# zamazincode/cv-diffusion-model

Measured on AMD Instinct MI355X. Metric: images/sec (whole node), 256×256 4-step LCM 'small'; PSNR vs CPU ref, higher is better.
Workload: dtype fp16; 1 GPU; variant=small, 256x256, batch=32/GPU, 4 LCM steps, fp16, 1xMI355X (BASELINE configs[1] per GPU); global_batch=32, parallelism=single GPU

## Files before the change

cv-diffusion-model_amd/_native.py:

```python
from __future__ import annotations

import ctypes as C
import os
from typing import List, Tuple

_HERE = os.path.dirname(os.path.abspath(__file__))
LIB_PATH = os.path.join(_HERE, "libllie_hip.so")

LLIE_F32, LLIE_F16, LLIE_BF16 = 0, 1, 2
LLIE_UNET, LLIE_IRB, LLIE_ATTN, LLIE_DOWN, LLIE_UP, LLIE_SE = 0, 1, 2, 3, 4, 5
ERR_ARG, ERR_SHAPE, ERR_CONFIG, ERR_KEY, ERR_NOT_LOADED, ERR_WORKSPACE, ERR_NO_DEVICE = -1, -2, -3, -4, -5, -6, -7
SAMPLER_LCM, SAMPLER_DDIM = 0, 1

EXPORTS = [
    "llie_last_error", "llie_version", "llie_create", "llie_destroy", "llie_num_params", "llie_param_info",
    "llie_load_param", "llie_params_loaded", "llie_workspace_bytes", "llie_unet_forward", "llie_module_forward",
    "llie_lcm_step", "llie_add_noise", "llie_enhance", "llie_algorithmic_bytes", "llie_flops",
    "llie_profile_begin", "llie_profile_end", "llie_enhance_workspace_bytes",
    "llie_preprocess_u8", "llie_postprocess_u8", "llie_profile_report", "llie_pw_gemm", "llie_pw_gemm_tile_rows", "llie_dwconv3x3", "llie_dwconv3x3_tiles", "llie_tune",
    "llie_grad_numel", "llie_param_grad_offset", "llie_train_workspace_bytes", "llie_unet_train_forward",
    "llie_unet_backward", "llie_module_backward", "llie_load_all", "llie_profile_dump", "llie_copy_probe", "llie_rw_probe", "llie_pw_expand", "llie_gram_stats", "llie_gram_part_floats", "llie_groupnorm_finalize", "llie_conv3x3", "llie_conv3x3_tiles", "llie_linattn", "llie_linattn_splits", "llie_se_mlp", "llie_film", "llie_refresh_params", "llie_path_bytes", "llie_time_embed", "llie_debug_irbx_stamps", "llie_debug_gemm_stamps", "llie_debug_pwx_stamps", "llie_graph_cache_entries", "llie_debug_conv_stamps", "llie_gram_finalize",
    "llie_optimizer_create", "llie_optimizer_destroy", "llie_optimizer_numel", "llie_optimizer_step",
    "llie_optimizer_step_amp",
    "llie_consistency_target", "llie_consistency_loss", "llie_ema_create", "llie_ema_update", "llie_ema_destroy",
    "llie_wgrad", "llie_wgrad_msplit", "llie_wgrad_partial_floats", "llie_dw_wgrad", "llie_dw_wgrad_strips",
    "llie_groupnorm_backward", "llie_groupnorm_backward_scratch_floats", "llie_linattn_backward", "llie_linattn_dkv_floats",
    "llie_upsample2x_backward", "llie_dilate2x", "llie_linear_dx", "llie_linear_dx_scratch_floats", "llie_linear_dw",
    "llie_final_bwd_data",
    "llie_dwconv3x3_backward", "llie_groupnorm_backward_from_slab", "llie_bias_grad", "llie_bias_grad_floats", "llie_pack_planes",
    "llie_add_into", "llie_sin_embed", "llie_pointwise_backward",
    "llie_tile_count", "llie_tile_origins", "llie_tile_gather_u8", "llie_tile_gather_f32", "llie_tile_blend_u8",
    "llie_tile_sync_step",
    "llie_aug_pair_u8", "llie_aug_synth_u8",
    "llie_image_metrics_scratch_bytes", "llie_image_metrics_f32", "llie_image_metrics_u8", "llie_comparison_grid_u8",
    "llie_upconv_fold_elems", "llie_upconv_fold_weights", "llie_conv3x3_upfold", "llie_conv3x3_upfold_tiles",
    "llie_expand_dw", "llie_expand_pool", "llie_expand_dw_project", "llie_expand_dw_project_skip", "llie_irbx_project_tiles",
    "llie_expand_stats", "llie_irbx_stats_rows",
    "llie_dwconv3x3_ex", "llie_dwconv3x3_strip_rows", "llie_last_kernel",
    "llie_init_conv", "llie_init_conv_tiles", "llie_init_conv_pack_bytes", "llie_final_conv", "llie_final_conv_pack_bytes",
    "llie_se_gate", "llie_affine_add", "llie_nchw_to_nhwc", "llie_nhwc_to_nchw", "llie_pw_gemm_dot",
    "llie_frame_shape_ok", "llie_frame_workspace_bytes", "llie_unet_forward_hw", "llie_enhance_hw",
    "llie_frame_pad", "llie_frame_load_u8", "llie_frame_store_u8",
    "llie_ssim_grad_scratch_bytes", "llie_ssim_grad_f32", "llie_x0_loss",
    "llie_train_shape_ok", "llie_unet_train_forward_hw", "llie_aug_pair_u8_hw", "llie_aug_synth_u8_hw",
    "llie_tile_gather_u8_hw", "llie_tile_gather_f32_hw", "llie_tile_blend_u8_hw", "llie_tile_sync_step_hw", "llie_frame_max_pixels",
]
K_GEMM, K_DW, K_CONV3, K_SE, K_OTHER = 1, 2, 4, 8, 16
PW_SIGMOID_BWD, PW_RELU6_BWD, PW_SILU_BWD, PW_SCALE = 0, 1, 2, 3


class GemmSeg(C.Structure):
    _fields_ = [("ptr", C.c_void_p), ("channels", C.c_int), ("scale", C.c_void_p), ("bias", C.c_void_p),
                ("affine_ld", C.c_int), ("act", C.c_int)]


class GnBackwardArgs(C.Structure):
    _fields_ = [("g", C.c_void_p), ("dz", C.c_void_p), ("x0", C.c_void_p), ("x1", C.c_void_p), ("c0", C.c_int), ("c1", C.c_int),
                ("scale", C.c_void_p), ("shift", C.c_void_p), ("act", C.c_int), ("mean", C.c_void_p), ("rstd", C.c_void_p),
                ("gamma", C.c_void_p), ("beta", C.c_void_p), ("film", C.c_void_p), ("film_stride", C.c_int64), ("dfilm", C.c_void_p),
                ("dfilm_stride", C.c_int64), ("dgamma", C.c_void_p), ("dbeta", C.c_void_p), ("add0", C.c_void_p), ("add1_0", C.c_void_p),
                ("add1_1", C.c_void_p), ("dx0", C.c_void_p), ("dx1", C.c_void_p), ("batch", C.c_int), ("pixels", C.c_int)]


class LibraryNotBuilt(RuntimeError):
    pass


class Config(C.Structure):
# ... 116 lines not shown
    L.llie_frame_workspace_bytes.restype = i64
    L.llie_unet_forward_hw.argtypes = [vp, vp, vp, vp, ci, vp, ci, ci, ci, vp, i64, vp]
    L.llie_enhance_hw.argtypes = [vp, vp, vp, vp, C.POINTER(StepCoef), ci, vp, vp, vp, ci, ci, ci, vp, i64, vp]
    L.llie_frame_pad.argtypes = [ci]
    L.llie_frame_load_u8.argtypes = [vp, ci, ci, vp, vp]
    L.llie_frame_store_u8.argtypes = [vp, ci, ci, vp, vp]
    L.llie_aug_pair_u8.argtypes = [vp, vp, ci, vp, ci, ci, ci, vp, vp, vp, vp, vp]
    L.llie_aug_synth_u8.argtypes = [vp, vp, ci, vp, ci, ci, ci, vp, vp, vp, vp, vp, vp]
    L.llie_aug_pair_u8_hw.argtypes = [vp, vp, ci, vp, ci, ci, ci, ci, vp, vp, vp, vp, vp]
    L.llie_aug_synth_u8_hw.argtypes = [vp, vp, ci, vp, ci, ci, ci, ci, vp, vp, vp, vp, vp, vp]
    L.llie_image_metrics_scratch_bytes.argtypes = [ci, ci, ci]
    L.llie_image_metrics_scratch_bytes.restype = i64
    L.llie_image_metrics_f32.argtypes = [vp, vp, ci, ci, ci, C.c_float, C.c_float, vp, vp, i64, vp]
    L.llie_image_metrics_u8.argtypes = [vp, vp, ci, ci, ci, vp, vp, i64, vp]
    L.llie_ssim_grad_scratch_bytes.argtypes = [ci, ci, ci]
    L.llie_ssim_grad_scratch_bytes.restype = i64
    L.llie_ssim_grad_f32.argtypes = [vp, vp, ci, ci, ci, C.c_float, C.c_float, vp, vp, vp, vp, i64, vp]
    L.llie_x0_loss.argtypes = [vp, vp, vp, vp, vp, ci, ci, C.c_float, C.c_float, vp, vp, ci, ci, ci, vp, i64, vp]
    L.llie_comparison_grid_u8.argtypes = [vp, vp, vp, ci, ci, ci, vp, vp]
    L.llie_pw_gemm.argtypes = [ci, C.POINTER(GemmSeg), ci, vp, vp, vp, vp, vp, ci, ci, ci, vp]
    L.llie_pw_gemm_tile_rows.argtypes = [ci]
    L.llie_pw_expand.argtypes = [ci, C.POINTER(GemmSeg), ci, vp, vp, vp, vp, ci, ci, ci, vp]
    L.llie_gram_stats.argtypes = [ci, vp, ci, vp, ci, vp, vp, ci, ci, vp, vp, vp, vp]
    L.llie_gram_part_floats.argtypes = [ci, ci]
    L.llie_gram_finalize.argtypes = [ci, vp, vp, ci, ci, vp, vp, vp, i64, C.c_float, C.c_float, ci, vp, vp, vp]
    L.llie_groupnorm_finalize.argtypes = [vp, ci, ci, vp, ci, ci, ci, ci, vp, vp, vp, i64, C.c_float, C.c_float, ci, vp, vp, vp]
    L.llie_conv3x3.argtypes = [ci, ci, vp, vp, vp, vp, vp, ci, ci, ci, ci, ci, vp]
    L.llie_conv3x3_tiles.argtypes = [ci, ci]
    L.llie_upconv_fold_elems.argtypes = [ci]
    L.llie_upconv_fold_elems.restype = i64
    L.llie_upconv_fold_weights.argtypes = [ci, vp, vp, ci, vp]
    L.llie_conv3x3_upfold.argtypes = [ci, vp, vp, vp, vp, vp, ci, ci, ci, ci, vp]
    L.llie_conv3x3_upfold_tiles.argtypes = [ci, ci]
    L.llie_linattn.argtypes = [ci, vp, vp, vp, ci, ci, ci, vp]
    L.llie_linattn_splits.argtypes = [ci]
    L.llie_se_mlp.argtypes = [ci, vp, ci, vp, vp, vp, vp, vp, vp, vp, ci, ci, ci, vp]
    L.llie_film.argtypes = [vp, vp, vp, vp, ci, ci, ci, vp]
    L.llie_gram_part_floats.restype = i64
    L.llie_dwconv3x3.argtypes = [ci, vp, vp, vp, vp, vp, vp, ci, ci, ci, ci, vp]
    L.llie_dwconv3x3_tiles.argtypes = [ci, ci]
    L.llie_dwconv3x3_ex.argtypes = [ci, vp, vp, vp, vp, vp, vp, vp, ci, ci, ci, ci, ci, vp]
    L.llie_dwconv3x3_strip_rows.argtypes = [ci, ci, ci, ci, ci]
    L.llie_init_conv_pack_bytes.argtypes = [ci, ci]
    L.llie_init_conv_pack_bytes.restype = i64
    L.llie_init_conv_tiles.argtypes = [ci, ci, ci]
    L.llie_init_conv.argtypes = [ci, vp, ci, vp, ci, vp, vp, vp, vp, ci, ci, ci, ci, ci, vp, i64, vp]
    L.llie_final_conv_pack_bytes.argtypes = [ci]
    L.llie_final_conv_pack_bytes.restype = i64
    L.llie_final_conv.argtypes = [ci, vp, vp, vp, vp, vp, vp, ci, ci, ci, ci, ci, ci, C.POINTER(StepCoef), vp, vp, vp, vp, vp, i64, vp]
    L.llie_se_gate.argtypes = [ci, vp, ci, vp, vp, vp, vp, vp, ci, ci, ci, ci, vp, vp, vp]
    L.llie_affine_add.argtypes = [ci, vp, vp, vp, vp, vp, vp, ci, ci, ci, vp]
    L.llie_nchw_to_nhwc.argtypes = [ci, vp, vp, vp, ci, ci, ci, ci, ci, vp]
    L.llie_nhwc_to_nchw.argtypes = [ci, vp, vp, ci, ci, ci, ci, ci, vp]
    L.llie_pw_gemm_dot.argtypes = [ci, C.POINTER(GemmSeg), ci, vp, vp, vp, vp, vp, ci, ci, ci, vp]
    L.llie_last_kernel.argtypes = []
    L.llie_last_kernel.restype = C.c_char_p
    L.llie_expand_dw.argtypes = [ci, vp, ci, vp, ci, vp, vp, vp, vp, vp, vp, vp, vp, ci, ci, ci, vp]
    L.llie_expand_pool.argtypes = [ci, vp, ci, vp, ci, vp, vp, vp, vp, vp, vp, vp, ci, ci, ci, vp]
    L.llie_expand_dw_project.argtypes = [ci, vp, ci, vp, vp, vp, vp, vp, vp, vp, vp, vp, vp, ci, ci, ci, vp]
    L.llie_expand_dw_project_skip.argtypes = [ci, vp, ci, vp, ci, vp, vp, vp, vp, vp, vp, vp, vp, ci, ci, vp, vp, ci, ci, ci, vp]
    L.llie_irbx_project_tiles.argtypes = [ci, ci]
    L.llie_expand_stats.argtypes = [ci, vp, ci, vp, ci, vp, vp, vp, vp, ci, ci, ci, vp]
    L.llie_irbx_stats_rows.argtypes = [ci]
    L.llie_tune.argtypes = [C.c_char_p, ci]
    L.llie_debug_irbx_stamps.argtypes = [C.POINTER(C.c_double)]
    L.llie_optimizer_create.argtypes = [C.POINTER(OptTensor), ci, C.POINTER(C.c_void_p)]
# ... 222 lines not shown
```

cv-diffusion-model_amd/csrc/engine.h:

```cpp
#pragma once
#include <hip/hip_runtime.h>

#include <algorithm>
#include <cmath>
#include <cstdarg>
#include <cstdio>
#include <cstdlib>
#include <cstring>
#include <map>
#include <tuple>
#include <string>
#include <vector>

#include "../../include/llie.h"
#include "kernels.h"

namespace llie {

void set_err(const char* fmt, ...);
inline hipStream_t hs(llie_stream stream) { return reinterpret_cast<hipStream_t>(stream); }

inline size_t elem_size(int dt) { return dt == LLIE_F32 ? 4 : 2; }
inline size_t align_up(size_t x, size_t a) { return (x + a - 1) / a * a; }

// ... 162 lines not shown
  struct GraphEntry { bool seen = false; hipGraphExec_t exec = nullptr; hipGraph_t graph = nullptr; uint64_t used = 0; };
  static constexpr size_t kMaxGraphs = 16;
  uint64_t graph_clock = 0;
  std::map<std::string, GraphEntry> graphs;
  std::map<std::tuple<int, int, int, int>, size_t> zneed;
  hipStream_t cap_stream = nullptr;
  hipStream_t side_stream = nullptr;
  hipEvent_t ev_fork = nullptr, ev_join = nullptr;
  hipStream_t branch_stream[llie::kMaxBranches] = {};
  hipEvent_t branch_join[llie::kMaxBranches] = {};
  int prof_mask = 0;
  struct ProfRec { int cls; int64_t bytes; hipEvent_t e0, e1; const char* name; char tag[56]; };
  std::vector<ProfRec> prof;
  std::vector<hipEvent_t> event_pool;
  hipEvent_t get_event() {
    if (!event_pool.empty()) { hipEvent_t e = event_pool.back(); event_pool.pop_back(); return e; }
    hipEvent_t e = nullptr;
    if (hipEventCreate(&e) != hipSuccess) return nullptr;
    return e;
  }
};

namespace llie {

struct Knobs {
  int use_irbx;
  int irbx_project;
  int gram;
  int nt_min_mb;
  int nt_mask;
  int se_mfma;
  int bwd_async;
  int upconv_fold;
  int enhance_split;
  int graph_max_steps;
  int epoch;
};
extern Knobs g_knobs;
constexpr int kGraphMaxSteps = 20;

enum IrbForm { kIrbUnfused, kIrbRecompute, kIrbProject };
struct IrbPath {
  IrbForm form;
  bool s6;
  bool fixtot;
  bool gram;
};
inline IrbPath irb_path(int dt, const IrbW& w, int c0, int H, int W, bool training) {
  IrbPath p{kIrbUnfused, !training && dt != LLIE_F32, !training && w.hid % 128 == 0, false};
  if (!p.fixtot || !g_knobs.use_irbx || w.hid != w.hid_r || w.cin != w.cin_r || !irbx_supported(dt, w.cin, c0, w.hid, H, W)) return p;
  p.gram = g_knobs.gram && (H * W >= 32768 || g_knobs.gram > 1) && gram_supported(dt, w.cin, c0, H * W);
  const int tail = g_knobs.irbx_project && w.cout == w.cout_r ? irbx_project_supported(dt, w.cin, c0, w.hid, w.cout, w.skip, H, W) : 0;
  p.form = tail && !(tail == kIrbxProjectSkip && g_knobs.irbx_project == 2) ? kIrbProject : kIrbRecompute;
  return p;
}

inline bool upconv_fold_supported(int dt, int Hi, int Wi, int C) {
  return g_knobs.upconv_fold && (C == 64 || C == 128) && conv3x3_upfold_ok(dt, Hi, Wi, C);
}

struct Exec {
  llie_ctx* c;
  Arena* ar;
  hipStream_t s;
  char* ws;
  bool dry;
  int B;
  int dt;
  hipError_t err = hipSuccess;
  static Exec planning(llie_ctx* c, Arena* ar, int B) { return Exec{c, ar, nullptr, nullptr, true, B, c->dt}; }
  static Exec live(llie_ctx* c, Arena* ar, llie_stream stream, void* ws, int B) {
    return Exec{c, ar, hs(stream), reinterpret_cast<char*>(ws), false, B, c->dt};
  }
  template <typename T = void> T* wptr(size_t off) const { return reinterpret_cast<T*>(c->blob + off); }
  template <typename T = void> T* p(size_t off) const {
    if (dry) return nullptr;
    return reinterpret_cast<T*>(ws + off);
  }
  void chk(hipError_t e) { if (e != hipSuccess && err == hipSuccess) err = e; }
  size_t es() const { return elem_size(dt); }
  FilmArgs film_args(size_t silu_temb, int rows, int T, size_t wf, size_t bf, size_t film, int F) const {
    FilmArgs fa{};
    fa.silu_temb = p<float>(silu_temb); fa.rows = rows; fa.T = T; fa.wf = wptr<float>(wf); fa.bf = wptr<float>(bf);
    fa.film = p<float>(film); fa.F = F;
    return fa;
  }
  int rc(bool backward = false) const;
};

int check_loaded(const llie_ctx* c);
int check_ready(const llie_ctx* c);
// ... 18 lines not shown
```

cv-diffusion-model_amd/csrc/forward.cpp:

```cpp
#include "engine.h"

using namespace llie;

namespace {

struct Run : Exec {
  Tape* tape = nullptr;
  char tag[56] = "";
  void rel(size_t off) { if (!tape) ar->free(off); }
  size_t zoff = 0, zcur = 0, zcap = 0;
  bool zcount = false;
  template <typename F> void zbegin(int H, int W, F&& forward_again) {
    if (tape || zcount) return;
    const auto key = std::make_tuple(B, H, W, g_knobs.epoch);
    auto it = c->zneed.find(key);
    if (it == c->zneed.end()) {
      size_t zbytes = 0;
      plan(c, B, forward_again, &zbytes);
      it = c->zneed.emplace(key, zbytes).first;
    }
    zcap = it->second;
    if (!zcap) return;
    zoff = ar->alloc(zcap);
    if (!dry) chk(launch_zero_fill(ws + zoff, (int64_t)zcap, s));
// ... 287 lines not shown
      a.qkv = p(qkv); a.B = B; a.N = N; a.heads = w.heads; a.kv = p<float>(kv); a.out = p(ao); a.nsplit = nsplit;
      timed(LLIE_K_OTHER, (int64_t)M * 2 * w.inner * (int64_t)es(), [&] { return launch_linattn_kv(dt, a, s); }, "linattn_kv_kernel");
      timed(LLIE_K_OTHER, (int64_t)M * 2 * w.inner * (int64_t)es(), [&] { return launch_linattn_out(dt, a, s); }, "linattn_out_kernel");
    }
    rel(qkv); rel(kv);
    Tens tmp = new_tens(x.C, H, W, pw_gemm_ntiles(N));
    if (!dry) {
      const GemmArgs g = gemm1(GemmSeg{p(ao), w.inner, nullptr, nullptr, 0, ACT_NONE}, wptr(w.w_out), p(tmp.off), p<float>(tmp.slab), M, x.C, w.inner, N);
      timed(LLIE_K_GEMM, ((int64_t)M * (x.C + w.inner) + (int64_t)w.inner * x.C) * (int64_t)es(), [&] { return launch_pw_gemm(dt, g, s); });
    }
    rel(ao);
    size_t as2, ab2;
    gn(tmp, nullptr, w.n2g, w.n2b, nullptr, 0, as2, ab2, &rec.n2);
    Tens y = new_tens(x.C, H, W, (N + kAffineTileRows - 1) / kAffineTileRows);
    if (!dry) {
      AffineAddArgs a{};
      a.x = p(tmp.off); a.as = p<float>(as2); a.ab = p<float>(ab2); a.res = p(x.off); a.y = p(y.off);
      a.stats = p<float>(y.slab); a.M = M; a.C = x.C; a.P = N;
      timed(LLIE_K_OTHER, 3LL * M * x.C * (int64_t)es(), [&] { return launch_affine_add(dt, a, s); }, "affine_add_kernel");
    }
    free_tens(tmp);
    rel(as2); rel(ab2);
    if (tape) {
      rec.w = (int)(&w - c->attns.data());
      rec.x = x; rec.qkv = qkv; rec.kv = kv; rec.ao = ao; rec.nsplit = nsplit; rec.tmp = tmp; rec.y = y;
      tape->ops.push_back({1, (int)tape->attns.size()});
      tape->attns.push_back(rec);
    }
    return y;
  }

  Tens conv3(const ConvW& w, const Tens& x, int mode) {
    const int Ho = mode == 0 ? x.H / 2 : x.H * 2, Wo = mode == 0 ? x.W / 2 : x.W * 2;
    const bool fold = mode == 1 && !tape && w.has_fold && upconv_fold_supported(dt, x.H, x.W, w.c);
    Tens y = new_tens(w.c, Ho, Wo, fold ? conv3x3_upfold_ntiles(Ho, Wo) : conv3x3_ntiles(Ho, Wo), w.c_r);
    Tens u;
    snprintf(tag, sizeof tag, "conv3 mode=%d C=%d %dx%d", mode, w.c, x.H, x.W);
    if (tape && mode == 1) {
      u.C = w.c; u.H = Ho; u.W = Wo; u.valid = true;
      u.off = ar->alloc((size_t)B * Ho * Wo * w.c * es());
    }
    if (!dry) {
      const Tens& in = u.valid ? u : x;
      Conv3Args a{};
      a.in = p(in.off); a.w = wptr(w.w); a.bias = wptr<float>(w.bias); a.out = p(y.off); a.stats = p<float>(y.slab);
      a.B = B; a.Hi = in.H; a.Wi = in.W; a.Cin = w.c; a.Cout = w.c; a.mode = u.valid ? 2 : mode;
      if (u.valid) {
        chk(launch_upsample2x(dt, p(x.off), p(u.off), B, x.H, x.W, w.c, s));
        timed(LLIE_K_CONV3, (2LL * B * w.c * Ho * Wo + 9LL * w.c * w.c) * (int64_t)es(), [&] { return launch_conv3x3(dt, a, s); });
      } else {
        a.nt = nt_store(16, (int64_t)B * Ho * Wo * w.c);
        if (fold) a.w = wptr(w.w_fold);
        timed(LLIE_K_CONV3, ((int64_t)B * w.c * ((int64_t)x.H * x.W + (int64_t)Ho * Wo) + 9LL * w.c * w.c) * (int64_t)es(),
              [&] { return fold ? launch_conv3x3_upfold(dt, a, s) : launch_conv3x3(dt, a, s); });
      }
    }
    if (tape) {
      ConvRec rec{};
      rec.w = mode == 0 ? (int)(&w - c->downs.data()) : (int)(&w - c->ups.data());
      rec.up = mode != 0; rec.x = x; rec.u = u; rec.y = y;
      tape->ops.push_back({2, (int)tape->convs.size()});
      tape->convs.push_back(rec);
    }
    return y;
  }

  Tens run_blocks(const std::vector<Block>& blocks, Tens h, const Tens* cat, const float* film, int64_t fstride,
                  bool keep_input) {
    bool first = true;
    for (const Block& b : blocks) {
      Tens y = b.kind == 0 ? irb(c->irbs[b.idx], h, first ? cat : nullptr, film, fstride) : attn(c->attns[b.idx], h);
      if (!(first && keep_input)) free_tens(h);
      h = y;
      first = false;
    }
    return h;
  }

  void unet(const float* lat, const float* cond, const int64_t* t, int uniform_t, float* eps, int H, int W, const FusedStep* fs = nullptr) {
    const llie_config& g = c->cfg;
    const int T = g.time_embed_dim, F = c->film_rows;
    const int rows = uniform_t ? 1 : B;
    zbegin(H, W, [&](Run& d) { d.unet(nullptr, nullptr, nullptr, uniform_t, nullptr, H, W); });
    const size_t temb = ar->alloc((size_t)rows * T * 4), stemb = ar->alloc((size_t)rows * T * 4);
    const size_t film = ar->alloc((size_t)rows * F * 4);
    if (!dry) {
      TimeArgs ta{};
// ... 241 lines not shown
```

cv-diffusion-model_amd/csrc/kernel_api.cpp:

```cpp
#include "engine.h"

using namespace llie;

static bool dtype_ok(int dtype) { return dtype >= 0 && dtype <= 2; }

int llie::kerr(const char* what, hipError_t e, int refuse_rc, const char* refuse_msg) {
  if (e == hipSuccess) return LLIE_OK;
  if (e == hipErrorInvalidValue && refuse_rc) {
    if (refuse_msg) set_err("%s: %s", what, refuse_msg);
    return refuse_rc;
  }
  set_err("%s: %s", what, hipGetErrorString(e));
  return (int)e;
}

static int to_segs(const llie_gemm_seg* segs, int nseg, GemmSeg* out) {
  int K = 0;
  for (int i = 0; i < nseg; ++i) {
    out[i] = GemmSeg{segs[i].ptr, segs[i].channels, segs[i].scale, segs[i].bias, segs[i].affine_ld, segs[i].act};
    K += segs[i].channels;
  }
  return K;
}

// ... 89 lines not shown
  a.eps = eps; a.as = scale_out; a.ab = shift_out; a.B = batch; a.post_scale = post_scale;
  return kerr("groupnorm_finalize", launch_gn_finalize(a, hs(stream)));
}
int llie_gram_finalize(int dtype, const float* gram_totals, const void* w_expand, int K, int pixels, const float* gamma, const float* beta,
                       const float* film, int64_t film_stride, float eps, float post_scale, int batch, float* scale_out, float* shift_out,
                       llie_stream stream) {
  if (!gram_totals || !w_expand || !gamma || !beta || !scale_out || !shift_out || batch <= 0 || pixels <= 0 || (K != 32 && K != 64 && K != 96) ||
      (dtype != 1 && dtype != 2))
    return LLIE_ERR_ARG;
  GramFinalizeArgs a{};
  a.gtot = gram_totals; a.w1 = w_expand; a.K = K; a.Chid = 4 * K; a.groups = 32; a.P = pixels; a.B = batch; a.gamma = gamma; a.beta = beta;
  a.film = film; a.film_stride = film_stride; a.eps = eps; a.as = scale_out; a.ab = shift_out; a.post_scale = post_scale;
  return kerr("gram_finalize", launch_gram_finalize(dtype, a, hs(stream)));
}
int llie_conv3x3(int dtype, int mode, const void* in, const void* w, const float* bias, void* out, float* stats, int batch, int Hi, int Wi,
                 int Cin, int Cout, llie_stream stream) {
  if (!in || !w || !out || dtype < 0 || dtype > 2 || mode < 0 || mode > 2) return LLIE_ERR_ARG;
  Conv3Args a{};
  a.in = in; a.w = w; a.bias = bias; a.out = out; a.stats = stats; a.B = batch; a.Hi = Hi; a.Wi = Wi; a.Cin = Cin; a.Cout = Cout; a.mode = mode;
  return kerr("conv3x3", launch_conv3x3(dtype, a, hs(stream)));
}
int llie_conv3x3_tiles(int Ho, int Wo) { return conv3x3_ntiles(Ho, Wo); }
int64_t llie_upconv_fold_elems(int C) { return C > 0 ? (int64_t)upconv_fold_elems(C) : LLIE_ERR_ARG; }
int llie_upconv_fold_weights(int dtype, const float* w_oihw, void* folded, int C, llie_stream stream) {
  if (!w_oihw || !folded || C < 1 || (dtype != 1 && dtype != 2)) return LLIE_ERR_ARG;
  return kerr("upconv_fold_weights", launch_upconv_fold(dtype, w_oihw, folded, C, hs(stream)));
}
int llie_conv3x3_upfold(int dtype, const void* in, const void* folded, const float* bias, void* out, float* stats, int batch, int Hi, int Wi,
                        int C, llie_stream stream) {
  if (!in || !folded || !out || (dtype != 1 && dtype != 2)) return LLIE_ERR_ARG;
  Conv3Args a{};
  a.in = in; a.w = folded; a.bias = bias; a.out = out; a.stats = stats; a.B = batch; a.Hi = Hi; a.Wi = Wi; a.Cin = C; a.Cout = C; a.mode = 1;
  return kerr("conv3x3_upfold", launch_conv3x3_upfold(dtype, a, hs(stream)));
}
int llie_conv3x3_upfold_tiles(int Ho, int Wo) { return conv3x3_upfold_ntiles(Ho, Wo); }
int llie_linattn_splits(int N) { return linattn_nsplit(N); }
int llie_linattn(int dtype, const void* qkv, float* kv_scratch, void* out, int batch, int N, int heads, llie_stream stream) {
  if (!qkv || !kv_scratch || !out || dtype < 0 || dtype > 2 || batch <= 0 || N <= 0 || heads <= 0) return LLIE_ERR_ARG;
  AttnArgs a{};
  a.qkv = qkv; a.B = batch; a.N = N; a.heads = heads; a.kv = kv_scratch; a.out = out; a.nsplit = linattn_nsplit(N);
  hipError_t e = launch_linattn_kv(dtype, a, hs(stream));
  if (e == hipSuccess) e = launch_linattn_out(dtype, a, hs(stream));
  return kerr("linattn", e);
}
int llie_se_mlp(int dtype, const float* pool_sums, int pixels, const void* w1, const float* b1, const void* w2, const float* b2, float* mean_scratch,
                float* hidden_scratch, float* gate, int batch, int C, int Cs, llie_stream stream) {
  if (!pool_sums || !w1 || !b1 || !w2 || !b2 || !mean_scratch || !hidden_scratch || !gate || dtype < 0 || dtype > 2 || batch <= 0 || C <= 0 || Cs <= 0)
    return LLIE_ERR_ARG;
  SeArgs a{};
  a.pool = pool_sums; a.ntiles = 1; a.P = pixels; a.w1 = w1; a.b1 = b1; a.w2 = w2; a.b2 = b2; a.mean = mean_scratch; a.hid = hidden_scratch; a.gate = gate;
  a.B = batch; a.C = C; a.Cs = Cs;
  hipError_t e = launch_se_fc1(dtype, a, hs(stream));
  if (e == hipSuccess) e = launch_se_fc2(dtype, a, hs(stream));
  return kerr("se_mlp", e);
}

static int64_t align16(int64_t n) { return (n + 15) & ~(int64_t)15; }
static bool conv_sizes_ok(int B, int H, int W) { return B > 0 && B <= 65535 && H > 0 && W > 0 && H % 8 == 0 && W % 8 == 0; }
int64_t llie_init_conv_pack_bytes(int Cin, int Cout) {
  if (Cin < 1 || Cin > 8 || Cout <= 0 || Cout % 32) return LLIE_ERR_ARG;
  return align16((int64_t)Cin * 9 * Cout * 4) + (int64_t)10 * Cout * 8 * 2;
}
int64_t llie_final_conv_pack_bytes(int C) {
  if (C <= 0 || C % 32) return LLIE_ERR_ARG;
  return (int64_t)9 * C * 4 * 4 + (int64_t)(C / 32) * 18 * 2 * 4 * 8 * 2;
}
// ... 680 lines not shown
```

cv-diffusion-model_amd/csrc/kernels.h:

```cpp
#pragma once
#include <hip/hip_runtime.h>
#include <stdint.h>

namespace llie {

enum Act : int { ACT_NONE = 0, ACT_RELU6 = 1, ACT_SILU = 2, ACT_RELU6_S6 = 3 };

void note_kernel(const char* name);
const char* last_kernel();

struct StatSrc {
  const float* slab;
  int ntiles;
  int ch;
};

struct GemmSeg {
  const void* ptr;
  int ch;
  const float* as;
  const float* ab;
  int aff_ld;
  int act;
};
// ... 181 lines not shown
};
hipError_t launch_init_conv(int dtype, const InitConvArgs& a, hipStream_t s);
int init_conv_ntiles(int H, int W, bool mfma);
struct StepCoef { float sa, sb, sap, sbp; int is_last; int vpred; int clamp_x0; int sampler; };
struct FinalConvArgs {
  const void* in; const float* as; const float* ab;
  const float* w; const float* bias;
  const void* wp;
  float* out;
  int B, H, W, C, Cout;
  int fuse_step;
  StepCoef coef;
  const float* sample; const float* noise; float* prev; float* clamped;
};
hipError_t launch_final_conv(int dtype, const FinalConvArgs& a, hipStream_t s);
struct Conv3Args {
  const void* in;
  const void* w;
  const float* bias;
  void* out;
  float* stats;
  int B, Hi, Wi, Cin, Cout;
  int mode;
  int nt;
  unsigned long long* stamps;
};
void conv3x3_stamp(int v);
hipError_t conv3x3_stamp_fetch(double* out8);
hipError_t launch_conv3x3(int dtype, const Conv3Args& a, hipStream_t s);
int conv3x3_ntiles(int Ho, int Wo);
bool conv3x3_upfold_ok(int dtype, int Hi, int Wi, int C);
hipError_t launch_conv3x3_upfold(int dtype, const Conv3Args& a, hipStream_t s);
int conv3x3_upfold_ntiles(int Ho, int Wo);
constexpr int kUpconvFoldSets = 64;
inline size_t upconv_fold_elems(int C) { return (size_t)kUpconvFoldSets * C * C; }

struct AttnArgs {
  const void* qkv; int B, N, heads;
  float* kv;
  void* out;
  int nsplit;
};
int linattn_nsplit(int N);
hipError_t launch_linattn_kv(int dtype, const AttnArgs& a, hipStream_t s);
hipError_t launch_linattn_out(int dtype, const AttnArgs& a, hipStream_t s);

struct AffineAddArgs {
  const void* x; const float* as; const float* ab; const void* res; void* y; float* stats;
  int M, C, P;
};
hipError_t launch_affine_add(int dtype, const AffineAddArgs& a, hipStream_t s);
constexpr int kAffineTileRows = 64;

hipError_t launch_nchw_to_nhwc(int dtype, const float* x, void* y, float* stats, int B, int C, int P, int Csrc,
                               int coff, hipStream_t s);
hipError_t launch_nhwc_to_nchw(int dtype, const void* x, float* y, int B, int C, int P, hipStream_t s, int Cdst = 0,
                               int coff = 0);

enum PKind : int { PK_F32, PK_MAT, PK_CONV3, PK_DW, PK_INIT, PK_FINAL };
struct LoadDesc {
  const float* src;
  PKind kind;
  int as_t;
  int rows, cols, ld, col0, O, I, Op, Ip;
  long long numel, dst, dst_t, dst_f;
  float fscale;
// ... 247 lines not shown
```

cv-diffusion-model_amd/csrc/tune.cpp:

```cpp
#include "engine.h"

using namespace llie;

static Knobs knob_defaults() {
  Knobs k{};
  k.use_irbx = getenv("LLIE_NO_IRBX") ? 0 : 1;
  k.irbx_project = 1;
  k.gram = 1;
  k.nt_min_mb = 100; k.nt_mask = 1;
  k.upconv_fold = 1;
  k.se_mfma = 1;
  k.bwd_async = 1;
  k.enhance_split = getenv("LLIE_ENHANCE_SPLIT") ? atoi(getenv("LLIE_ENHANCE_SPLIT")) : 2;
  k.graph_max_steps = kGraphMaxSteps;
  k.epoch = 0;
  return k;
}
Knobs llie::g_knobs = knob_defaults();

static hipError_t elapsed_ms(const llie_ctx::ProfRec& r, float* ms) {
  hipError_t e = hipEventSynchronize(r.e1);
  if (e == hipSuccess) e = hipEventElapsedTime(ms, r.e0, r.e1);
  if (e != hipSuccess) set_err("profile: %s", hipGetErrorString(e));
  return e;
}

static int read_stamps(double* out, hipError_t (*fetch)(double*)) {
  if (!out) return LLIE_ERR_ARG;
  hipError_t e = hipDeviceSynchronize();
  if (e == hipSuccess) e = fetch(out);
  return e == hipSuccess ? LLIE_OK : LLIE_ERR_ARG;
}

extern "C" {

int llie_tune(const char* knob, int value) {
  if (!knob) return LLIE_ERR_ARG;
  ++g_knobs.epoch;
  if (!strcmp(knob, "gemm_bk")) { pw_gemm_force_bk(value); return LLIE_OK; }
  if (!strcmp(knob, "se_mfma")) { g_knobs.se_mfma = value; return LLIE_OK; }
  if (!strcmp(knob, "nt_min_mb")) { g_knobs.nt_min_mb = value; return LLIE_OK; }
  if (!strcmp(knob, "nt_mask")) { g_knobs.nt_mask = value; return LLIE_OK; }
  if (!strcmp(knob, "upconv_fold")) { g_knobs.upconv_fold = value != 0; return LLIE_OK; }
  if (!strcmp(knob, "gram")) { g_knobs.gram = value; return LLIE_OK; }
  if (!strcmp(knob, "irbx")) { g_knobs.use_irbx = value != 0; return LLIE_OK; }
  if (!strcmp(knob, "irbx_project")) { g_knobs.irbx_project = value < 0 || value > 2 ? 1 : value; return LLIE_OK; }
  if (!strcmp(knob, "irbx_dbuf")) { irbx_tune(value); return LLIE_OK; }
  if (!strcmp(knob, "irbx_stamp")) { irbx_stamp(value); return LLIE_OK; }
  if (!strcmp(knob, "irbx_grid")) { irbx_grid(0, value); return LLIE_OK; }
  if (!strcmp(knob, "irbx_grid2")) { irbx_grid(2, value); return LLIE_OK; }
  if (!strcmp(knob, "irbx_grid4")) { irbx_grid(4, value); return LLIE_OK; }
  if (!strcmp(knob, "irbx_grid6")) { irbx_grid(6, value); return LLIE_OK; }
  if (!strcmp(knob, "conv_stamp")) { conv3x3_stamp(value); return LLIE_OK; }
  if (!strcmp(knob, "gemm_stamp")) { pw_gemm_stamp(value); return LLIE_OK; }
  if (!strcmp(knob, "pwx")) { pw_expand_enable(value); return LLIE_OK; }
  if (!strcmp(knob, "pwx_stamp")) { pw_expand_debug(value); return LLIE_OK; }
  if (!strcmp(knob, "bwd_async")) { g_knobs.bwd_async = value; return LLIE_OK; }
  if (!strcmp(knob, "enhance_split")) { g_knobs.enhance_split = value; return LLIE_OK; }
  if (!strcmp(knob, "graph_max_steps")) { g_knobs.graph_max_steps = value > 0 ? value : kGraphMaxSteps; return LLIE_OK; }
  return LLIE_ERR_ARG;
}

int llie_debug_gemm_stamps(double* out3) { return read_stamps(out3, pw_gemm_stamp_fetch); }
int llie_debug_pwx_stamps(double* out4) { return read_stamps(out4, pw_expand_stamp_fetch); }
int llie_debug_conv_stamps(double* out8) { return read_stamps(out8, conv3x3_stamp_fetch); }
int llie_debug_irbx_stamps(double* out10) { return read_stamps(out10, irbx_stamp_fetch); }

int llie_profile_begin(llie_ctx* c, int class_mask) {
  if (!c) return LLIE_ERR_ARG;
  for (auto& r : c->prof) { c->event_pool.push_back(r.e0); c->event_pool.push_back(r.e1); }
  c->prof.clear();
  c->prof_mask = class_mask;
  return LLIE_OK;
}

int llie_profile_end(llie_ctx* c, int kernel_class, double* total_ms, int64_t* launches, int64_t* alg_bytes) {
// ... 56 lines not shown
```

include/llie.h:

```cpp
#ifndef LLIE_H_
#define LLIE_H_

#include <stddef.h>
#include <stdint.h>

#ifdef __cplusplus
extern "C" {
#endif

typedef struct llie_ctx llie_ctx;
typedef void* llie_stream;

enum llie_status {
  LLIE_OK = 0,
  LLIE_ERR_ARG = -1,
  LLIE_ERR_SHAPE = -2,
  LLIE_ERR_CONFIG = -3,
  LLIE_ERR_KEY = -4,
  LLIE_ERR_NOT_LOADED = -5,
  LLIE_ERR_WORKSPACE = -6,
  LLIE_ERR_NO_DEVICE = -7
};

enum llie_dtype { LLIE_F32 = 0, LLIE_F16 = 1, LLIE_BF16 = 2 };
// ... 183 lines not shown
                           int64_t scratch_bytes, llie_stream stream);
int llie_image_metrics_u8(const uint8_t* a, const uint8_t* b, int batch, int H, int W, double* out3, void* scratch,
                          int64_t scratch_bytes, llie_stream stream);

int64_t llie_ssim_grad_scratch_bytes(int batch, int H, int W);
int llie_ssim_grad_f32(const float* a, const float* b, int batch, int H, int W, float lo, float hi, const float* upstream,
                       float* ssim_out, float* da, void* scratch, int64_t scratch_bytes, llie_stream stream);
int llie_x0_loss(const float* out, const float* x_t, const float* normal, const int64_t* t, const float* alphas_cumprod, int table_n,
                 int velocity, float lambda_s, float lambda_1, float* loss_out, float* d_out, int batch, int H, int W, void* scratch,
                 int64_t scratch_bytes, llie_stream stream);

int llie_comparison_grid_u8(const float* low, const float* enhanced, const float* normal, int n, int H, int W, uint8_t* grid,
                            llie_stream stream);

typedef struct llie_gemm_seg {
  const void* ptr; int channels; const float* scale; const float* bias; int affine_ld; int act;
} llie_gemm_seg;
int llie_pw_gemm(int dtype, const llie_gemm_seg* segs, int nseg, const void* w, const float* bias, const void* residual,
                 void* out, float* stats, int M, int N, int P, llie_stream stream);
int llie_pw_gemm_tile_rows(int P);
int llie_pw_expand(int dtype, const llie_gemm_seg* segs, int nseg, const float* w32, void* wpack, void* out, float* stats,
                   int M, int N, int P, llie_stream stream);
int llie_groupnorm_finalize(const float* slab0, int ntiles0, int ch0, const float* slab1, int ntiles1, int ch1, int groups, int pixels,
                            const float* gamma, const float* beta, const float* film, int64_t film_stride, float eps, float post_scale,
                            int batch, float* scale_out, float* shift_out, llie_stream stream);
int llie_conv3x3(int dtype, int mode, const void* in, const void* w, const float* bias, void* out, float* stats, int batch, int Hi, int Wi,
                 int Cin, int Cout, llie_stream stream);
int llie_conv3x3_tiles(int Ho, int Wo);
int64_t llie_upconv_fold_elems(int C);
int llie_upconv_fold_weights(int dtype, const float* w_oihw, void* folded, int C, llie_stream stream);
int llie_conv3x3_upfold(int dtype, const void* in, const void* folded, const float* bias, void* out, float* stats, int batch, int Hi, int Wi,
                        int C, llie_stream stream);
int llie_conv3x3_upfold_tiles(int Ho, int Wo);
int llie_linattn(int dtype, const void* qkv, float* kv_scratch, void* out, int batch, int N, int heads, llie_stream stream);
int llie_linattn_splits(int N);
int llie_se_mlp(int dtype, const float* pool_sums, int pixels, const void* w1, const float* b1, const void* w2, const float* b2, float* mean_scratch,
                float* hidden_scratch, float* gate, int batch, int C, int Cs, llie_stream stream);
int llie_film(const float* silu_temb, const float* wf, const float* bf, float* film, int rows, int T, int F, llie_stream stream);

int64_t llie_init_conv_pack_bytes(int Cin, int Cout);
int llie_init_conv_tiles(int H, int W, int mfma);
int llie_init_conv(int dtype, const float* x0, int c0, const float* x1, int c1, const float* w_oihw, const float* bias, void* out, float* stats,
                   int batch, int H, int W, int Cout, int use_mfma, void* pack, int64_t pack_bytes, llie_stream stream);
int64_t llie_final_conv_pack_bytes(int C);
int llie_final_conv(int dtype, const void* in, const float* scale, const float* shift, const float* w_oihw, const float* bias, float* out,
                    int batch, int H, int W, int C, int Cout, int use_mfma, const llie_step_coef* coef, const float* sample, const float* noise,
                    float* prev, float* clamped, void* pack, int64_t pack_bytes, llie_stream stream);
int llie_se_gate(int dtype, const unsigned long long* totals, int pixels, const void* w1, const float* b1, const void* w2, const float* b2,
                 float* gate, int batch, int C, int Cs, int path, float* hidden_scratch, long long* pre_scratch, llie_stream stream);
int llie_affine_add(int dtype, const void* x, const float* scale, const float* shift, const void* res, void* y, float* stats, int M, int C, int P,
                    llie_stream stream);
int llie_nchw_to_nhwc(int dtype, const float* x, void* y, float* stats, int batch, int C, int P, int Csrc, int coff, llie_stream stream);
int llie_nhwc_to_nchw(int dtype, const void* x, float* y, int batch, int C, int P, int Cdst, int coff, llie_stream stream);
int llie_pw_gemm_dot(int dtype, const llie_gemm_seg* segs, int nseg, const void* w, const float* bias, const void* dot, void* out,
                     float* stats, int M, int N, int P, llie_stream stream);

int llie_wgrad(int dtype, const void* g, int N, const llie_gemm_seg* segs, int nseg, int batch, int Ho, int Wo, int Hi, int Wi, int stride,
               int dy, int dx, int ntap, int nstore, int kstore, float* partial, int64_t partial_floats, float* out, int64_t ldn, int64_t ldk,
               int64_t off, int msplit, llie_stream stream);
int llie_wgrad_msplit(int dtype, int batch, int pixels, int N, int K, int ntap, int ragged_rule);
int64_t llie_wgrad_partial_floats(int msplit, int N, int K, int ntap);
int llie_dw_wgrad(int dtype, const void* g, const float* gs, const float* gb, const void* h, const float* scale, const float* shift,
                  float* partial, float* out, int batch, int H, int W, int C, llie_stream stream);
int llie_dw_wgrad_strips(int H, int W);
typedef struct llie_gn_backward_args {
  const void* g; void* dz;
// ... 95 lines not shown
```

Before: 1247 images/sec.

## Add low-resolution upsample-conv kernel for 256-channel up blocks

```diff
diff --git a/cv-diffusion-model_amd/_native.py b/cv-diffusion-model_amd/_native.py
--- a/cv-diffusion-model_amd/_native.py
+++ b/cv-diffusion-model_amd/_native.py
@@ -33,7 +33,7 @@
     "llie_tile_sync_step",
     "llie_aug_pair_u8", "llie_aug_synth_u8",
     "llie_image_metrics_scratch_bytes", "llie_image_metrics_f32", "llie_image_metrics_u8", "llie_comparison_grid_u8",
-    "llie_upconv_fold_elems", "llie_upconv_fold_weights", "llie_conv3x3_upfold", "llie_conv3x3_upfold_tiles",
+    "llie_upconv_fold_elems", "llie_upconv_fold_weights", "llie_conv3x3_upfold", "llie_conv3x3_upfold_tiles", "llie_conv3x3_uplow",
     "llie_expand_dw", "llie_expand_pool", "llie_expand_dw_project", "llie_expand_dw_project_skip", "llie_irbx_project_tiles",
     "llie_expand_stats", "llie_irbx_stats_rows",
     "llie_dwconv3x3_ex", "llie_dwconv3x3_strip_rows", "llie_last_kernel",
@@ -216,6 +216,7 @@
     L.llie_upconv_fold_weights.argtypes = [ci, vp, vp, ci, vp]
     L.llie_conv3x3_upfold.argtypes = [ci, vp, vp, vp, vp, vp, ci, ci, ci, ci, vp]
     L.llie_conv3x3_upfold_tiles.argtypes = [ci, ci]
+    L.llie_conv3x3_uplow.argtypes = [ci, vp, vp, vp, vp, vp, ci, ci, ci, ci, vp]
     L.llie_linattn.argtypes = [ci, vp, vp, vp, ci, ci, ci, vp]
     L.llie_linattn_splits.argtypes = [ci]
     L.llie_se_mlp.argtypes = [ci, vp, ci, vp, vp, vp, vp, vp, vp, vp, ci, ci, ci, vp]
diff --git a/cv-diffusion-model_amd/csrc/engine.h b/cv-diffusion-model_amd/csrc/engine.h
--- a/cv-diffusion-model_amd/csrc/engine.h
+++ b/cv-diffusion-model_amd/csrc/engine.h
@@ -218,6 +218,7 @@
   int se_mfma;
   int bwd_async;
   int upconv_fold;
+  int upconv_lowres;
   int enhance_split;
   int graph_max_steps;
   int epoch;
@@ -243,6 +244,9 @@
 
 inline bool upconv_fold_supported(int dt, int Hi, int Wi, int C) {
   return g_knobs.upconv_fold && (C == 64 || C == 128) && conv3x3_upfold_ok(dt, Hi, Wi, C);
+}
+inline bool upconv_lowres_supported(int dt, int Hi, int Wi, int C) {
+  return g_knobs.upconv_lowres && g_knobs.upconv_fold && (C == 256 || g_knobs.upconv_lowres > 1) && conv3x3_uplow_ok(dt, Hi, Wi, C);
 }
 
 struct Exec {
diff --git a/cv-diffusion-model_amd/csrc/forward.cpp b/cv-diffusion-model_amd/csrc/forward.cpp
--- a/cv-diffusion-model_amd/csrc/forward.cpp
+++ b/cv-diffusion-model_amd/csrc/forward.cpp
@@ -343,8 +343,9 @@
 
   Tens conv3(const ConvW& w, const Tens& x, int mode) {
     const int Ho = mode == 0 ? x.H / 2 : x.H * 2, Wo = mode == 0 ? x.W / 2 : x.W * 2;
-    const bool fold = mode == 1 && !tape && w.has_fold && upconv_fold_supported(dt, x.H, x.W, w.c);
-    Tens y = new_tens(w.c, Ho, Wo, fold ? conv3x3_upfold_ntiles(Ho, Wo) : conv3x3_ntiles(Ho, Wo), w.c_r);
+    const bool lowres = mode == 1 && !tape && w.c == w.c_r && upconv_lowres_supported(dt, x.H, x.W, w.c);
+    const bool fold = !lowres && mode == 1 && !tape && w.has_fold && upconv_fold_supported(dt, x.H, x.W, w.c);
+    Tens y = new_tens(w.c, Ho, Wo, lowres || fold ? conv3x3_upfold_ntiles(Ho, Wo) : conv3x3_ntiles(Ho, Wo), w.c_r);
     Tens u;
     snprintf(tag, sizeof tag, "conv3 mode=%d C=%d %dx%d", mode, w.c, x.H, x.W);
     if (tape && mode == 1) {
@@ -363,7 +364,7 @@
         a.nt = nt_store(16, (int64_t)B * Ho * Wo * w.c);
         if (fold) a.w = wptr(w.w_fold);
         timed(LLIE_K_CONV3, ((int64_t)B * w.c * ((int64_t)x.H * x.W + (int64_t)Ho * Wo) + 9LL * w.c * w.c) * (int64_t)es(),
-              [&] { return fold ? launch_conv3x3_upfold(dt, a, s) : launch_conv3x3(dt, a, s); });
+              [&] { return lowres ? launch_conv3x3_uplow(dt, a, s) : (fold ? launch_conv3x3_upfold(dt, a, s) : launch_conv3x3(dt, a, s)); });
       }
     }
     if (tape) {
diff --git a/cv-diffusion-model_amd/csrc/kernel_api.cpp b/cv-diffusion-model_amd/csrc/kernel_api.cpp
--- a/cv-diffusion-model_amd/csrc/kernel_api.cpp
+++ b/cv-diffusion-model_amd/csrc/kernel_api.cpp
@@ -145,6 +145,13 @@
   Conv3Args a{};
   a.in = in; a.w = folded; a.bias = bias; a.out = out; a.stats = stats; a.B = batch; a.Hi = Hi; a.Wi = Wi; a.Cin = C; a.Cout = C; a.mode = 1;
   return kerr("conv3x3_upfold", launch_conv3x3_upfold(dtype, a, hs(stream)));
+}
+int llie_conv3x3_uplow(int dtype, const void* in, const void* w9, const float* bias, void* out, float* stats, int batch, int Hi, int Wi, int C,
+                       llie_stream stream) {
+  if (!in || !w9 || !out || (dtype != 1 && dtype != 2)) return LLIE_ERR_ARG;
+  Conv3Args a{};
+  a.in = in; a.w = w9; a.bias = bias; a.out = out; a.stats = stats; a.B = batch; a.Hi = Hi; a.Wi = Wi; a.Cin = C; a.Cout = C; a.mode = 1;
+  return kerr("conv3x3_uplow", launch_conv3x3_uplow(dtype, a, hs(stream)));
 }
 int llie_conv3x3_upfold_tiles(int Ho, int Wo) { return conv3x3_upfold_ntiles(Ho, Wo); }
 int llie_linattn_splits(int N) { return linattn_nsplit(N); }
diff --git a/cv-diffusion-model_amd/csrc/kernels.h b/cv-diffusion-model_amd/csrc/kernels.h
--- a/cv-diffusion-model_amd/csrc/kernels.h
+++ b/cv-diffusion-model_amd/csrc/kernels.h
@@ -237,6 +237,8 @@
 bool conv3x3_upfold_ok(int dtype, int Hi, int Wi, int C);
 hipError_t launch_conv3x3_upfold(int dtype, const Conv3Args& a, hipStream_t s);
 int conv3x3_upfold_ntiles(int Ho, int Wo);
+bool conv3x3_uplow_ok(int dtype, int Hi, int Wi, int C);
+hipError_t launch_conv3x3_uplow(int dtype, const Conv3Args& a, hipStream_t s);
 constexpr int kUpconvFoldSets = 64;
 inline size_t upconv_fold_elems(int C) { return (size_t)kUpconvFoldSets * C * C; }
 
diff --git a/cv-diffusion-model_amd/csrc/tune.cpp b/cv-diffusion-model_amd/csrc/tune.cpp
--- a/cv-diffusion-model_amd/csrc/tune.cpp
+++ b/cv-diffusion-model_amd/csrc/tune.cpp
@@ -9,6 +9,7 @@
   k.gram = 1;
   k.nt_min_mb = 100; k.nt_mask = 1;
   k.upconv_fold = 1;
+  k.upconv_lowres = 1;
   k.se_mfma = 1;
   k.bwd_async = 1;
   k.enhance_split = getenv("LLIE_ENHANCE_SPLIT") ? atoi(getenv("LLIE_ENHANCE_SPLIT")) : 2;
@@ -42,6 +43,7 @@
   if (!strcmp(knob, "nt_min_mb")) { g_knobs.nt_min_mb = value; return LLIE_OK; }
   if (!strcmp(knob, "nt_mask")) { g_knobs.nt_mask = value; return LLIE_OK; }
   if (!strcmp(knob, "upconv_fold")) { g_knobs.upconv_fold = value != 0; return LLIE_OK; }
+  if (!strcmp(knob, "upconv_lowres")) { g_knobs.upconv_lowres = value < 0 || value > 2 ? 1 : value; return LLIE_OK; }
   if (!strcmp(knob, "gram")) { g_knobs.gram = value; return LLIE_OK; }
   if (!strcmp(knob, "irbx")) { g_knobs.use_irbx = value != 0; return LLIE_OK; }
   if (!strcmp(knob, "irbx_project")) { g_knobs.irbx_project = value < 0 || value > 2 ? 1 : value; return LLIE_OK; }
diff --git a/cv-diffusion-model_amd/csrc/upconv.hip b/cv-diffusion-model_amd/csrc/upconv.hip
--- /dev/null
+++ b/cv-diffusion-model_amd/csrc/upconv.hip
@@ -0,0 +1,272 @@
+#include <string>
+#include <type_traits>
+
+#include "common.h"
+#include "kernels.h"
+
+namespace llie {
+
+namespace {
+
+__host__ __device__ constexpr float up_coef(int a, int r, int d) {
+  const int q = a + r - 1, i2 = (q + 2) / 2 - 1, a2 = (q + 2) % 2;
+  return d == i2 ? 0.75f : (d == (a2 ? i2 + 1 : i2 - 1) ? 0.25f : 0.f);
+}
+
+template <typename T> __device__ __forceinline__ uint32_t pack2(float lo, float hi) {
+  typedef T t2 __attribute__((ext_vector_type(2)));
+  t2 o;
+  o[0] = (T)lo;
+  o[1] = (T)hi;
+  return *reinterpret_cast<uint32_t*>(&o);
+}
+template <typename T> __device__ __forceinline__ float dot2_pair(uint32_t x, uint32_t y, float c) {
+  if constexpr (std::is_same<T, half_t>::value) {
+    return __builtin_amdgcn_fdot2(*reinterpret_cast<const f16x2*>(&x), *reinterpret_cast<const f16x2*>(&y), c, false);
+  } else {
+    typedef __bf16 b2 __attribute__((ext_vector_type(2)));
+    return __builtin_amdgcn_fdot2_f32_bf16(*reinterpret_cast<const b2*>(&x), *reinterpret_cast<const b2*>(&y), c, false);
+  }
+}
+
+constexpr int kUlNT = 512, kUlCc = 32;
+constexpr int kUlPH = 10, kUlPW = 18, kUlHalo = kUlPH * kUlPW, kUlHaloPad = 192;
+constexpr int kUlWRows = 3 * kUlCc;
+constexpr int kUlZPitch = 36;
+
+template <typename T, int C> constexpr size_t uplow_x_bytes() { return (size_t)kUlHalo * (C + 8) * sizeof(T); }
+template <typename T, int C> constexpr size_t uplow_lds() {
+  constexpr size_t w = (size_t)kUlWRows * (C + 8) * sizeof(T), z = (size_t)2 * kUlHalo * kUlZPitch * 4;
+  return uplow_x_bytes<T, C>() + (w > z ? w : z);
+}
+
+template <typename T, int C>
+__global__ void __launch_bounds__(kUlNT) conv3x3_uplow_kernel(const Conv3Args a) {
+  constexpr int NT = kUlNT, VEC = Elem<T>::VEC, XP = C + 8, TH = 8, TW = 16, PW = kUlPW, Cc = kUlCc, NW = NT / 64;
+  constexpr int CV = C / VEC;
+  constexpr int W_ITEMS = kUlWRows * CV, W_PER = (W_ITEMS + NT - 1) / NT;
+  typedef typename Elem<T>::vec_t vec_t;
+  static_assert(VEC == 8 && C % 32 == 0, "2-byte types only");
+
+  extern __shared__ __align__(16) unsigned char smem[];
+  T* sX = reinterpret_cast<T*>(smem);
+  T* sW = reinterpret_cast<T*>(smem + uplow_x_bytes<T, C>());
+  uint32_t* sP = reinterpret_cast<uint32_t*>(smem + uplow_x_bytes<T, C>());
+  uint32_t* sQ = sP + kUlHalo * kUlZPitch;
+  float* red = reinterpret_cast<float*>(smem);
+
+  const int tid = threadIdx.x, lane = tid & 63, wave = __builtin_amdgcn_readfirstlane(tid >> 6);
+  const int pg = wave & 3, rh = wave >> 2;
+  const int H = a.Hi, W = a.Wi, Ho = 2 * H, Wo = 2 * W;
+  const int TX = W / TW, tiles = TX * (H / TH), nbk = C / Cc;
+  int bid = blockIdx.x;
+  const int nblk = bid % nbk; bid /= nbk;
+  const int b = bid % a.B, tile = bid / a.B;
+  const int iy0 = (tile / TX) * TH, ix0 = (tile % TX) * TW, n0 = nblk * Cc;
+  const T* in = reinterpret_cast<const T*>(a.in) + (size_t)b * H * W * C;
+  const T* wbase = reinterpret_cast<const T*>(a.w);
+
+  vec_t wreg[W_PER];
+  auto load_w = [&](int r) {
+#pragma unroll
+    for (int it = 0; it < W_PER; ++it) {
+      const int i = tid + it * NT;
+      if (W_ITEMS % NT == 0 || i < W_ITEMS) {
+        const int n = i / CV, kv = (i % CV) * VEC;
+        wreg[it] = ld_vec<T>(wbase + ((size_t)(3 * r + (n >> 5)) * C + n0 + (n & 31)) * C + kv);
+      }
+    }
+  };
+  auto store_w = [&]() {
+#pragma unroll
+    for (int it = 0; it < W_PER; ++it) {
+      const int i = tid + it * NT;
+      if (W_ITEMS % NT == 0 || i < W_ITEMS) st_vec<T>(sW + (i / CV) * XP + (i % CV) * VEC, wreg[it]);
+    }
+  };
+  load_w(0);
+#pragma unroll 4
+  for (int i = tid; i < kUlHalo * CV; i += NT) {
+    const int hp = i / CV, kv = (i % CV) * VEC;
+    const int gy = min(max(iy0 - 1 + hp / PW, 0), H - 1), gx = min(max(ix0 - 1 + hp % PW, 0), W - 1);
+    st_vec<T>(sX + hp * XP + kv, ld_vec<T>(in + ((size_t)gy * W + gx) * C + kv));
+  }
+  store_w();
+
+  int xrow[3];
+#pragma unroll
+  for (int blk = 0; blk < 3; ++blk) xrow[blk] = min(pg * 48 + blk * 16 + (lane & 15), kUlHalo - 1) * XP + 8 * (lane >> 4);
+  const int wrow = (rh * 16 + (lane & 15)) * XP + 8 * (lane >> 4);
+
+  const int px = tid >> 2, cg = tid & 3, py = px >> 4, pxx = px & 15;
+  const int gi = iy0 + py, gj = ix0 + pxx;
+  const float mr0 = gi == 0 ? 0.f : 1.f, mr2 = gi == H - 1 ? 0.f : 1.f, mc0 = gj == 0 ? 0.f : 1.f, mc2 = gj == W - 1 ? 0.f : 1.f;
+  uint32_t kP[2][3], kQ[2][3];
+#pragma unroll
+  for (int bb = 0; bb < 2; ++bb)
+#pragma unroll
+    for (int e = 0; e < 3; ++e) {
+      kP[bb][e] = pack2<T>(up_coef(bb, 0, e - 1) * (bb == 0 ? mc0 : 1.f), up_coef(bb, 1, e - 1));
+      kQ[bb][e] = pack2<T>(e == 2 ? up_coef(bb, 1, e - 1) : 0.f, up_coef(bb, 2, e - 1) * (bb == 1 ? mc2 : 1.f));
+    }
+  float y[2][2][VEC];
+#pragma unroll
+  for (int e = 0; e < VEC; ++e) {
+    const float bv = a.bias ? a.bias[n0 + cg * VEC + e] : 0.f;
+    y[0][0][e] = bv; y[0][1][e] = bv; y[1][0][e] = bv; y[1][1][e] = bv;
+  }
+  wg_barrier();
+
+#pragma unroll
+  for (int r = 0; r < 3; ++r) {
+    f32x4acc acc[3][3];
+#pragma unroll
+    for (int s = 0; s < 3; ++s)
+#pragma unroll
+      for (int blk = 0; blk < 3; ++blk) acc[s][blk] = f32x4acc{0.f, 0.f, 0.f, 0.f};
+#pragma unroll 2
+    for (int c0 = 0; c0 < C; c0 += 32) {
+      vec_t af[3], xb[3];
+#pragma unroll
+      for (int s = 0; s < 3; ++s) af[s] = ld_vec<T>(sW + s * Cc * XP + wrow + c0);
+#pragma unroll
+      for (int blk = 0; blk < 3; ++blk) xb[blk] = ld_vec<T>(sX + xrow[blk] + c0);
+#pragma unroll
+      for (int s = 0; s < 3; ++s)
+#pragma unroll
+        for (int blk = 0; blk < 3; ++blk) acc[s][blk] = mfma16x16<T>(af[s], xb[blk], acc[s][blk]);
+    }
+    wg_barrier();
+#pragma unroll
+    for (int blk = 0; blk < 3; ++blk) {
+      const int hp = pg * 48 + blk * 16 + (lane & 15), o = hp * kUlZPitch + rh * 16 + 4 * (lane >> 4);
+      u32x4 p, q;
+#pragma unroll
+      for (int i = 0; i < 4; ++i) {
+        p[i] = pack2<T>(acc[0][blk][i], acc[1][blk][i]);
+        q[i] = pack2<T>(acc[1][blk][i], acc[2][blk][i]);
+      }
+      if (hp < kUlHalo) {
+        *reinterpret_cast<u32x4*>(sP + o) = p;
+        *reinterpret_cast<u32x4*>(sQ + o) = q;
+      }
+    }
+    wg_barrier();
+    if (r < 2) load_w(r + 1);
+#pragma unroll
+    for (int d = -1; d <= 1; ++d) {
+      if (up_coef(0, r, d) == 0.f && up_coef(1, r, d) == 0.f) continue;
+      float hh[2][VEC];
+#pragma unroll
+      for (int e = 0; e < 3; ++e) {
+        const int o = ((py + 1 + d) * PW + pxx + e) * kUlZPitch + cg * VEC;
+        uint32_t zp[VEC], zq[VEC];
+        if (e < 2) {
+          const u32x4 v0 = *reinterpret_cast<const u32x4*>(sP + o), v1 = *reinterpret_cast<const u32x4*>(sP + o + 4);
+#pragma unroll
+          for (int k = 0; k < 4; ++k) { zp[k] = v0[k]; zp[4 + k] = v1[k]; }
+        }
+        if (e > 0) {
+          const u32x4 v0 = *reinterpret_cast<const u32x4*>(sQ + o), v1 = *reinterpret_cast<const u32x4*>(sQ + o + 4);
+#pragma unroll
+          for (int k = 0; k < 4; ++k) { zq[k] = v0[k]; zq[4 + k] = v1[k]; }
+        }
+#pragma unroll
+        for (int bb = 0; bb < 2; ++bb)
+#pragma unroll
+          for (int k = 0; k < VEC; ++k) {
+            float h = e == 0 ? 0.f : hh[bb][k];
+            if (e < 2) h = dot2_pair<T>(zp[k], kP[bb][e], h);
+            if (e > 0) h = dot2_pair<T>(zq[k], kQ[bb][e], h);
+            hh[bb][k] = h;
+          }
+      }
+#pragma unroll
+      for (int aa = 0; aa < 2; ++aa) {
+        if (up_coef(aa, r, d) == 0.f) continue;
+        const float cr = up_coef(aa, r, d) * (aa == 0 && r == 0 ? mr0 : (aa == 1 && r == 2 ? mr2 : 1.f));
+#pragma unroll
+        for (int bb = 0; bb < 2; ++bb)
+#pragma unroll
+          for (int k = 0; k < VEC; ++k) y[aa][bb][k] = __builtin_fmaf(hh[bb][k], cr, y[aa][bb][k]);
+      }
+    }
+    if (r < 2) {
+      wg_barrier();
+      store_w();
+      wg_barrier();
+    }
+  }
+
+  T* outp = reinterpret_cast<T*>(a.out) + (size_t)b * Ho * Wo * C + n0 + cg * VEC;
+  float v[64];
+#pragma unroll
+  for (int aa = 0; aa < 2; ++aa)
+#pragma unroll
+    for (int bb = 0; bb < 2; ++bb) {
+      const vec_t ov = f32_to_vec<T>(y[aa][bb]);
+      st_vec_pol<T>(outp + ((size_t)(2 * gi + aa) * Wo + 2 * gj + bb) * C, ov, a.nt != 0);
+#pragma unroll
+      for (int e = 0; e < VEC; ++e) {
+        const float q = (float)ov[e];
+        v[(aa * 2 + bb) * 16 + e] = q;
+        v[(aa * 2 + bb) * 16 + 8 + e] = q * q;
+      }
+    }
+  if (!a.stats) return;
+  {
+    const bool h4 = lane & 4, h8 = lane & 8, h16 = lane & 16, h32 = lane & 32;
+#pragma unroll
+    for (int i = 0; i < 32; ++i) v[i] = (h4 ? v[32 + i] : v[i]) + __shfl_xor(h4 ? v[i] : v[32 + i], 4, 64);
+#pragma unroll
+    for (int i = 0; i < 16; ++i) v[i] = (h8 ? v[16 + i] : v[i]) + __shfl_xor(h8 ? v[i] : v[16 + i], 8, 64);
+#pragma unroll
+    for (int i = 0; i < 8; ++i) v[i] = (h16 ? v[8 + i] : v[i]) + __shfl_xor(h16 ? v[i] : v[8 + i], 16, 64);
+#pragma unroll
+    for (int i = 0; i < 4; ++i) v[i] = (h32 ? v[4 + i] : v[i]) + __shfl_xor(h32 ? v[i] : v[4 + i], 32, 64);
+    const int base = (h4 ? 32 : 0) + (h8 ? 16 : 0) + (h16 ? 8 : 0) + (h32 ? 4 : 0);
+#pragma unroll
+    for (int i = 0; i < 4; ++i) red[(wave * 4 + cg) * 64 + base + i] = v[i];
+  }
+  wg_barrier();
+  if (tid < 4 * 64) {
+    const int idx = tid & 63, g = tid >> 6;
+    float t = 0.f;
+#pragma unroll
+    for (int w = 0; w < NW; ++w) t += red[(w * 4 + g) * 64 + idx];
+    const int phase = idx >> 4, which = (idx >> 3) & 1, ch = n0 + g * VEC + (idx & 7);
+    a.stats[((size_t)((b * tiles + tile) * 4 + phase) * 2 + which) * C + ch] = t;
+  }
+}
+
+template <typename T, int C>
+hipError_t launch_uplow_cfg(const Conv3Args& a, hipStream_t s) {
+  constexpr size_t lds = uplow_lds<T, C>();
+  static_assert(lds <= 160 * 1024, "LDS of a CU");
+  static std::atomic<uint64_t> attr_done{0};
+  if (hipError_t e = ensure_max_lds(reinterpret_cast<const void*>(&conv3x3_uplow_kernel<T, C>), (int)lds, attr_done); e != hipSuccess) return e;
+  const unsigned grid = (unsigned)(a.B * (a.Hi / 8) * (a.Wi / 16) * (C / kUlCc));
+  static const std::string name = std::string("conv3x3_upfold_kernel<") + TypeName<T>::value + ", " + std::to_string(C) + ", lowres>";
+  note_kernel(name.c_str());
+  hipLaunchKernelGGL((conv3x3_uplow_kernel<T, C>), dim3(grid), dim3(kUlNT), lds, s, a);
+  return hipGetLastError();
+}
+template <typename T>
+hipError_t launch_uplow_t(const Conv3Args& a, hipStream_t s) {
+  if (a.Cin == 64) return launch_uplow_cfg<T, 64>(a, s);
+  if (a.Cin == 128) return launch_uplow_cfg<T, 128>(a, s);
+  return launch_uplow_cfg<T, 256>(a, s);
+}
+
+}
+
+bool conv3x3_uplow_ok(int dtype, int Hi, int Wi, int C) {
+  return (dtype == 1 || dtype == 2) && Hi > 0 && Wi > 0 && Hi % 8 == 0 && Wi % 16 == 0 && (C == 64 || C == 128 || C == 256);
+}
+
+hipError_t launch_conv3x3_uplow(int dtype, const Conv3Args& a, hipStream_t s) {
+  if (a.Cin != a.Cout || a.B < 1 || !conv3x3_uplow_ok(dtype, a.Hi, a.Wi, a.Cin)) return hipErrorInvalidValue;
+  return dtype == 1 ? launch_uplow_t<half_t>(a, s) : launch_uplow_t<bf16_t>(a, s);
+}
+
+}
diff --git a/include/llie.h b/include/llie.h
--- a/include/llie.h
+++ b/include/llie.h
@@ -239,6 +239,8 @@
 int llie_conv3x3_upfold(int dtype, const void* in, const void* folded, const float* bias, void* out, float* stats, int batch, int Hi, int Wi,
                         int C, llie_stream stream);
 int llie_conv3x3_upfold_tiles(int Ho, int Wo);
+int llie_conv3x3_uplow(int dtype, const void* in, const void* w9, const float* bias, void* out, float* stats, int batch, int Hi, int Wi, int C,
+                       llie_stream stream);
 int llie_linattn(int dtype, const void* qkv, float* kv_scratch, void* out, int batch, int N, int heads, llie_stream stream);
 int llie_linattn_splits(int N);
 int llie_se_mlp(int dtype, const float* pool_sums, int pixels, const void* w1, const float* b1, const void* w2, const float* b2, float* mean_scratch,
```

Result: no change. 1257 images/sec (median of 6 runs) (+0.9%).
